# rlangefe/pygemma

Hardware: AMD Instinct MI355X
Metric: SNPs/sec (whole node) at n=10,000 c=5; K-eigendecomp wallclock (higher is better)
Workload: dtype i8x3->i32 MFMA (genotype codes exact, integer accumulation exact; U as 24-bit fixed point per eigenvector in three int8 planes) rotation + f64 Gram/sweeps (f32 rounding points of the reference)

## Files before the change

pygemma_amd/csrc/assoc.hip:

```cpp
#include "common.hpp"

#include <cmath>

namespace pg {

constexpr int NLAM = 11;
#ifndef PG_ASSOC_WPB
#define PG_ASSOC_WPB 2
#endif
constexpr int WPB = PG_ASSOC_WPB;
#define PG_MINV 1e-35f
#ifndef PG_FUSE_PQ_MAX
#define PG_FUSE_PQ_MAX 36
#endif
#ifndef PG_FUSE_PQR_MAX
#define PG_FUSE_PQR_MAX 28
#endif
#ifndef PG_PFD
#define PG_PFD 2
#endif
#ifndef PG_CHUNK_MIN_NP
#define PG_CHUNK_MIN_NP 80
#endif
#ifndef PG_SCAN_NV
#define PG_SCAN_NV 96
#endif
#ifndef PG_SWEEP_LDS_MIN_SLOTS
#define PG_SWEEP_LDS_MIN_SLOTS 3
#endif
#ifndef PG_PHENO_SPLIT_XE
#define PG_PHENO_SPLIT_XE 26
#endif
#ifndef PG_WAVES
#define PG_WAVES 2
#endif
#ifndef PG_ASSOC_FINAL_P
#define PG_ASSOC_FINAL_P 1
#endif
#ifndef PG_ASSOC_NEWTON_REUSE
#define PG_ASSOC_NEWTON_REUSE 1
#endif
#ifndef PG_REUSE_MAX_SLOTS
#define PG_REUSE_MAX_SLOTS 4
#endif

__host__ __device__ constexpr size_t assoc_sav_doubles(int sav_slots) { return sav_slots ? (size_t)2 * (2 * sav_slots + 1) * 64 : 0; }
__host__ __device__ constexpr size_t assoc_per_wave_bytes(int M, bool sweep_lds, int sav_slots, size_t evalout_bytes, int n_vals)
{
    return (((sweep_lds ? (size_t)3 * M * 8 : 0) + assoc_sav_doubles(sav_slots) * 8 + (size_t)NLAM * 2 * M * 8 + NLAM * evalout_bytes + 2 * NLAM * 4 +
             (size_t)n_vals * 4) + 15) & ~(size_t)15;
}

struct AssocParams {
    int n, npad, c, niter, nu, grid, rowf;
    long long p, ldx;
    const float *xr;
    const float *fixed;
    float *htab;
    double *fixg;
    double *t1tab;
    float *ldHtab;
    float lam11[NLAM];
    float logl_c;
    const int *leaf, *node, *level, *chunk;
    int n_leaf, n_level, n_chunk, n_vals;
    float *beta, *se, *tau, *lam;
    double *F;
    unsigned long long *stats;
    unsigned *trace;
    unsigned long long *passes;
    int lrt, nhalf;
    float ml_c;
    float *lalt, *lamalt;
    const double *xbuf;
    int xe, xcol;
};

struct EvalOut { float yPy, yPPy, yPPPy, trP, trPP, ld, Pxx_c, Pyx_c, sh, shh; };

__device__ __forceinline__ float hinv_f32(float lam, float d)
{
    const float x = __fadd_rn(__fmul_rn(lam, d), 1.0f);
    const float r0 = __builtin_amdgcn_rcpf(x);
    float r = __builtin_fmaf(__builtin_fmaf(-x, r0, 1.0f), r0, r0);
    if (__builtin_expect(!(x < 0x1p126f), 0)) r = __fdiv_rn(1.0f, x);
    return r;
}

__device__ __forceinline__ float np_logf(float x)
{
    const float p1 = 9.999999999999998702752e-01f, p2 = 2.112677543073053063722e+00f,
                p3 = 1.480000633576506585156e+00f, p4 = 3.808837741388407920751e-01f,
                p5 = 2.589979117907922693523e-02f;
    const float q1 = 2.612677543073109236779e+00f, q2 = 2.453006071784736363091e+00f,
                q3 = 9.864942958519418960339e-01f, q4 = 1.546476374983906719538e-01f,
                q5 = 5.875095403124574342950e-03f;
    if (__builtin_expect(!(x > 0.0f) || x == INFINITY, 0)) return (x != x) ? x : (x < 0.0f ? NAN : (x == 0.0f ? -INFINITY : x));
    unsigned u = __float_as_uint(x);
    int e = (int)((u >> 23) & 0xff) - 126;
    float m = __uint_as_float((u & 0x007fffffu) | 0x3f000000u);
    float ef = (float)e;
    if (m <= 0.70710678118f) { m = __fadd_rn(m, m); ef = __fsub_rn(ef, 1.0f); }
    float t = __fsub_rn(m, 1.0f);
    float den = fmaf(q5, t, q4);
    den = fmaf(den, t, q3); den = fmaf(den, t, q2); den = fmaf(den, t, q1); den = fmaf(den, t, 1.0f);
    float num = fmaf(p5, t, p4);
    num = fmaf(num, t, p3); num = fmaf(num, t, p2); num = fmaf(num, t, p1); num = fmaf(num, t, 0.0f);
    float poly = __fdiv_rn(num, den);
    return fmaf(ef, 0.693147180559945309417232121458176568f, poly);
}

__device__ __forceinline__ double bfly(double v)
{
#pragma unroll
// ... 136 lines not shown
        const bool b = (lane & s) != 0;
#pragma unroll
        for (int m = 0; m < NVP / (2 * s); m++) {
            const double keep = b ? v[2 * m + 1] : v[2 * m];
            const double send = b ? v[2 * m] : v[2 * m + 1];
            v[m] = keep + __shfl_xor(send, s, 64);
        }
    }
    double x = v[0];
#pragma unroll
    for (int s = NVP; s < 64; s <<= 1) x += __shfl_xor(x, s, 64);
    return x;
}

template <int C, int SL = 0>
__device__ __forceinline__ void scatter_entries(const double (&acc)[Shape<C>::NP], int lane, double (&out)[Shape<C>::SLOTS])
{
    constexpr int NV = Shape<C>::slot_nv(SL), NVP = next_pow2(NV);
    double t[NVP];
#pragma unroll
    for (int k = 0; k < NVP; k++) t[k] = (k < NV) ? acc[64 * SL + k] : 0.0;
    out[SL] = reduce_scatter<NVP>(t, lane);
    if constexpr (SL + 1 < Shape<C>::SLOTS) scatter_entries<C, SL + 1>(acc, lane, out);
}

template <int C> struct Own {
    int e[Shape<C>::SLOTS], r[Shape<C>::SLOTS], c[Shape<C>::SLOTS];
    bool valid[Shape<C>::SLOTS];
    __device__ __forceinline__ void init(int lane)
    {
#pragma unroll
        for (int sl = 0; sl < Shape<C>::SLOTS; sl++) {
            const int nv = Shape<C>::slot_nv(sl), k = lane % next_pow2(nv);
            valid[sl] = k < nv;
            e[sl] = valid[sl] ? 64 * sl + k : 0;
            int rr = 0;
            while ((rr + 1) * (rr + 2) / 2 <= e[sl]) rr++;
            r[sl] = rr; c[sl] = e[sl] - rr * (rr + 1) / 2;
        }
    }
};

template <int SLOTS>
__device__ __forceinline__ double gather(const double (&X)[SLOTS], int es)
{
    double v = __shfl(X[0], es & 63, 64);
#pragma unroll
    for (int sl = 1; sl < SLOTS; sl++) { const double w = __shfl(X[sl], es & 63, 64); v = ((es >> 6) == sl) ? w : v; }
    return v;
}

__device__ __forceinline__ void wave_lds_sync();

template <int C, int PW>
__device__ __forceinline__ void lane_sweeps(double (&P)[Shape<C>::SLOTS], double (&Q)[Shape<C>::SLOTS], double (&R)[Shape<C>::SLOTS],
                                            const Own<C> &own, double t1, double t2, int lane, EvalOut &o, double *piv)
{
    constexpr int M = Shape<C>::M, NP = Shape<C>::NP, SLOTS = Shape<C>::SLOTS;
    static_assert(PW == PW_P || PW == PW_PQ || PW == PW_PQR, "powers");
    constexpr bool DQ = (PW & 2) != 0, FULL = (PW & 4) != 0;
    constexpr bool VIA_LDS = Shape<C>::SWEEP_LDS;
    if (own.valid[0] && own.e[0] == 0) P[0] = dmaxf(P[0], PG_MINV);
    double trP = t1, trPP = t2, apiv = 1.0;
    for (int i = 1; i < M; i++) {
        const int q = i - 1, eqq = tri(q, q);
        double a, b = 0.0, e = 0.0;
        double ur[SLOTS], uc[SLOTS], vr[SLOTS], vc[SLOTS], wr[SLOTS], wc[SLOTS];
        bool act[SLOTS];
        if constexpr (VIA_LDS) {
#pragma unroll
            for (int sl = 0; sl < SLOTS; sl++)
                if (own.valid[sl] && own.c[sl] == q) {
                    piv[own.r[sl]] = P[sl];
                    if (DQ) piv[M + own.r[sl]] = Q[sl];
                    if (FULL) piv[2 * M + own.r[sl]] = R[sl];
                }
            wave_lds_sync();
            a = piv[q];
            if (DQ) b = piv[M + q];
            if (FULL) e = piv[2 * M + q];
#pragma unroll
            for (int sl = 0; sl < SLOTS; sl++) {
                act[sl] = own.valid[sl] && own.c[sl] >= i;
                const int rr = act[sl] ? own.r[sl] : q, cc = act[sl] ? own.c[sl] : q;
                ur[sl] = piv[rr]; uc[sl] = piv[cc];
                if (DQ) { vr[sl] = piv[M + rr]; vc[sl] = piv[M + cc]; }
                if (FULL) { wr[sl] = piv[2 * M + rr]; wc[sl] = piv[2 * M + cc]; }
            }
            wave_lds_sync();
        } else {
            a = gather<SLOTS>(P, eqq);
            if (DQ) b = gather<SLOTS>(Q, eqq);
            if (FULL) e = gather<SLOTS>(R, eqq);
#pragma unroll
            for (int sl = 0; sl < SLOTS; sl++) {
                act[sl] = own.valid[sl] && own.c[sl] >= i;
                const int er = act[sl] ? tri(own.r[sl], q) : 0, ec = act[sl] ? tri(own.c[sl], q) : 0;
                ur[sl] = gather<SLOTS>(P, er); uc[sl] = gather<SLOTS>(P, ec);
                if (DQ) { vr[sl] = gather<SLOTS>(Q, er); vc[sl] = gather<SLOTS>(Q, ec); }
                if (FULL) { wr[sl] = gather<SLOTS>(R, er); wc[sl] = gather<SLOTS>(R, ec); }
            }
        }
        if (lane == q) apiv = a;
        const double a2 = a * a, ia = -1.0 / a, ba2 = b / a2;
        if constexpr (FULL) {
            const double ba = b / a;
            trPP = (trPP + ba * ba) - 2 * (e / a);
            const double a3 = a2 * a, b2 = b * b;
            const double cR = (e / a2) - (b2 / a3);
#pragma unroll
            for (int sl = 0; sl < SLOTS; sl++)
                if (act[sl]) {
                    double s1 = fma(cR * uc[sl], ur[sl], R[sl]);
                    double s2 = fma(ia * uc[sl], wr[sl], 0.0); s2 = fma(ia * wc[sl], ur[sl], s2);
                    double s3 = fma(ia * vc[sl], vr[sl], 0.0);
                    double s4 = fma(ba2 * uc[sl], vr[sl], 0.0); s4 = fma(ba2 * vc[sl], ur[sl], s4);
                    double rn = ((s1 + s2) + s3) + s4;
                    if (own.r[sl] == i && own.c[sl] == i) rn = dmaxf(rn, PG_MINV);
                    R[sl] = rn;
                }
        }
        if constexpr (DQ) {
            trP = trP - b / a;
#pragma unroll
            for (int sl = 0; sl < SLOTS; sl++)
                if (act[sl]) {
                    double s1 = fma(ba2 * uc[sl], ur[sl], Q[sl]);
                    double s2 = fma(ia * uc[sl], vr[sl], 0.0); s2 = fma(ia * vc[sl], ur[sl], s2);
                    double qn = s1 + s2;
                    double pn = fma(ia * uc[sl], ur[sl], P[sl]);
                    if (own.r[sl] == i && own.c[sl] == i) { qn = dmaxf(qn, PG_MINV); pn = dmaxf(pn, PG_MINV); }
                    Q[sl] = qn; P[sl] = pn;
                }
        } else {
#pragma unroll
            for (int sl = 0; sl < SLOTS; sl++)
                if (act[sl]) {
                    double pn = fma(ia * uc[sl], ur[sl], P[sl]);
                    if (own.r[sl] == i && own.c[sl] == i) pn = dmaxf(pn, PG_MINV);
                    P[sl] = pn;
                }
        }
        if (i == M - 2) { o.Pxx_c = (float)gather<SLOTS>(P, tri(M - 2, M - 2)); o.Pyx_c = (float)gather<SLOTS>(P, tri(M - 1, M - 2)); }
    }
    const double lg = log(apiv);
    float ld = 0.0f;
    for (int q = 0; q < M - 1; q++) ld = (float)((double)ld + __shfl(lg, q, 64));
    o.yPy = (float)gather<SLOTS>(P, NP - 1);
    o.yPPy = DQ ? (float)gather<SLOTS>(Q, NP - 1) : 0.0f;
    o.yPPPy = FULL ? (float)gather<SLOTS>(R, NP - 1) : 0.0f;
    o.trP = DQ ? (float)trP : 0.0f;
    o.trPP = FULL ? (float)trPP : 0.0f;
    o.ld = ld;
    o.sh = (float)t1;
    o.shh = FULL ? (float)t2 : 0.0f;
}

template <int C> struct Elem {
    static constexpr int S4 = (C + 2 + 3) / 4;
    float4 row[S4];
    float x;
};
template <int C, bool HASX = true>
__device__ __forceinline__ void load_elem(const AssocParams &pr, const float *xrow, int i, Elem<C> &e)
{
    const float4 *src = reinterpret_cast<const float4 *>(pr.fixed + (size_t)i * pr.rowf);
#pragma unroll
    for (int k = 0; k < Elem<C>::S4; k++) e.row[k] = src[k];
    const int ic = min(i, pr.n - 1);
    e.x = HASX ? xrow[ic] : 0.0f;
}
constexpr int PFD = PG_PFD;
template <class E, int PF = PFD, class LoadF, class BodyF>
__device__ __forceinline__ void pipelined(int niter, LoadF &&ld, BodyF &&body)
{
    E buf[PF];
#pragma unroll
    for (int d = 0; d < PF; d++) ld(buf[d], d < niter ? d : niter - 1);
    for (int it = 0; it < niter; it += PF) {
#pragma unroll
        for (int d = 0; d < PF; d++) {
            if (it + d < niter) body(buf[d], it + d);
            const int nx = it + d + PF;
            ld(buf[d], nx < niter ? nx : niter - 1);
        }
    }
}
template <int C>
__device__ __forceinline__ void unpack_elem(const AssocParams &pr, const Elem<C> &e, int i, float &d, float (&col)[C + 2])
{
    float buf[4 * Elem<C>::S4];
#pragma unroll
    for (int k = 0; k < Elem<C>::S4; k++) {
        buf[4 * k] = e.row[k].x; buf[4 * k + 1] = e.row[k].y; buf[4 * k + 2] = e.row[k].z; buf[4 * k + 3] = e.row[k].w;
    }
    d = buf[0];
#pragma unroll
    for (int j = 0; j < C; j++) col[j] = buf[1 + j];
    col[C] = e.x;
    col[C + 1] = buf[C + 1];
// ... 113 lines not shown
        if constexpr (DR) slot_passes<C, 3, true, 0, EL>(pr, xrow, lam, lane, nullptr, R, t2);
    } else if constexpr (MASK == PW_PQR && Shape<C>::FUSE_PQR) {
        gram_pass<C, 7, true, EL>(pr, xrow, lam, lane, nullptr, P, Q, R, t1, t2);
    } else if constexpr (DP && DQ && Shape<C>::FUSE_PQ) {
        gram_pass<C, 3, true, EL>(pr, xrow, lam, lane, nullptr, P, Q, R, t1, t2);
        if constexpr (DR) gram_pass<C, 4, true, EL>(pr, xrow, lam, lane, nullptr, P, Q, R, t1, t2);
    } else {
        if constexpr (DP) gram_pass<C, 1, true, EL>(pr, xrow, lam, lane, nullptr, P, Q, R, t1, t2);
        if constexpr (DQ) gram_pass<C, 2, true, EL>(pr, xrow, lam, lane, nullptr, P, Q, R, t1, t2);
        if constexpr (DR) gram_pass<C, 4, true, EL>(pr, xrow, lam, lane, nullptr, P, Q, R, t1, t2);
    }
}

template <int C, int PW, class EL = WaldElem<C>>
__device__ __forceinline__ void eval_specific(const AssocParams &pr, typename EL::Row xrow, float lam, int lane, const Own<C> &own, EvalOut &o,
                                              double *piv)
{
    constexpr int SLOTS = Shape<C>::SLOTS;
    double P[SLOTS], Q[SLOTS], R[SLOTS], t1 = 0.0, t2 = 0.0;
#pragma unroll
    for (int sl = 0; sl < SLOTS; sl++) { Q[sl] = 0.0; R[sl] = 0.0; }
    gram_powers<C, PW, EL>(pr, xrow, lam, lane, P, Q, R, t1, t2);
    lane_sweeps<C, PW>(P, Q, R, own, t1, t2, lane, o, piv);
}

template <int C>
__global__ __launch_bounds__(64) void setup_tabs_kernel(AssocParams pr)
{
    constexpr int NP = Shape<C>::NP, SLOTS = Shape<C>::SLOTS;
    extern __shared__ float smem_f[];
    const int t = blockIdx.x, lane = threadIdx.x;
    const float lam = pr.lam11[t];
    Own<C> own;
    own.init(lane);
    double P[SLOTS], Q[SLOTS], R[SLOTS], t1 = 0.0, t2 = 0.0;
    if constexpr (Shape<C>::CHUNKED) {
        double tq = 0.0;
        slot_passes<C, 1, false>(pr, nullptr, lam, lane, pr.htab + (size_t)t * pr.npad, P, t1);
        slot_passes<C, 2, false>(pr, nullptr, lam, lane, nullptr, Q, tq);
    } else if constexpr (Shape<C>::FUSE_PQ) {
        gram_pass<C, 3, false>(pr, nullptr, lam, lane, pr.htab + (size_t)t * pr.npad, P, Q, R, t1, t2);
    } else {
        gram_pass<C, 1, false>(pr, nullptr, lam, lane, pr.htab + (size_t)t * pr.npad, P, Q, R, t1, t2);
        gram_pass<C, 2, false>(pr, nullptr, lam, lane, nullptr, P, Q, R, t1, t2);
    }
#pragma unroll
    for (int sl = 0; sl < SLOTS; sl++)
        if (own.valid[sl]) {
            pr.fixg[((size_t)t * 2 + 0) * NP + own.e[sl]] = P[sl];
            pr.fixg[((size_t)t * 2 + 1) * NP + own.e[sl]] = Q[sl];
        }
    float ldH = device_logdet_H(pr, lam, lane, smem_f);
    if (lane == 0) { pr.t1tab[t] = t1; pr.ldHtab[t] = ldH; }
}

template <int C, int GG>
__device__ __forceinline__ void scan_accumulate(const AssocParams &pr, const float *xrow, int t0, int lane, double *xent)
{
    constexpr int M = Shape<C>::M, NV = GG * 2 * M;
    constexpr int NV0 = NV < 64 ? NV : 64, NV1 = NV > 64 ? NV - 64 : 0;
    constexpr int NVP0 = next_pow2(NV0), NVP1 = next_pow2(NV1 > 0 ? NV1 : 1);
    static_assert(NV <= 128, "scan group too large");
    double acc[NV0 == 64 ? 64 + NVP1 : NVP0];
#pragma unroll
    for (int k = 0; k < (NV0 == 64 ? 64 + NVP1 : NVP0); k++) acc[k] = 0.0;
    struct SE { Elem<C> e; float h[GG]; };
    pipelined<SE>(pr.niter, [&](SE &q, int it) {
        const int i = it * 64 + lane;
        load_elem<C>(pr, xrow, i, q.e);
#pragma unroll
        for (int g = 0; g < GG; g++) q.h[g] = pr.htab[(size_t)(t0 + g) * pr.npad + i];
    }, [&](const SE &q, int it) {
        const int i = it * 64 + lane;
        float d, colf[M];
        unpack_elem<C>(pr, q.e, i, d, colf);
        const double xd = (double)colf[C];
        double z[M];
#pragma unroll
        for (int k = 0; k <= C; k++) z[k] = xd * (double)colf[k];
        z[C + 1] = (double)colf[C + 1] * xd;
#pragma unroll
        for (int g = 0; g < GG; g++) {
            const double hd = (double)q.h[g];
            const double h2 = hd * hd;
#pragma unroll
            for (int k = 0; k <= C + 1; k++) {
                acc[g * 2 * M + k] = fma(hd, z[k], acc[g * 2 * M + k]);
                acc[g * 2 * M + M + k] = fma(h2, z[k], acc[g * 2 * M + M + k]);
            }
        }
    });
    {
        double t[NVP0];
#pragma unroll
        for (int k = 0; k < NVP0; k++) t[k] = acc[k];
        const double tot = reduce_scatter<NVP0>(t, lane);
        const int idx = lane % NVP0;
        if (idx < NV0 && lane < NVP0) xent[t0 * 2 * M + idx] = tot;
    }
    if constexpr (NV1 > 0) {
        double t[NVP1];
#pragma unroll
        for (int k = 0; k < NVP1; k++) t[k] = acc[64 + k];
        const double tot = reduce_scatter<NVP1>(t, lane);
        const int idx = lane % NVP1;
        if (idx < NV1 && lane < NVP1) xent[t0 * 2 * M + 64 + idx] = tot;
// ... 120 lines not shown
        if (fabs(fblk) < fabs(fcur)) {
            xpre = xcur; xcur = xblk; xblk = xpre;
            fpre = fcur; fcur = fblk; fblk = fpre;
        }
        delta = (xtol + rtol * fabs(xcur)) / 2;
        sbis = (xblk - xcur) / 2;
        if (fcur == 0 || fabs(sbis) < delta) return xcur;
        if (fabs(spre) > delta && fabs(fcur) < fabs(fpre)) {
            if (xpre == xblk) {
                stry = -fcur * (xcur - xpre) / (fcur - fpre);
            } else {
                dpre = (fpre - fcur) / (xpre - xcur);
                dblk = (fblk - fcur) / (xblk - xcur);
                stry = -fcur * (fblk * dblk - fpre * dpre) / (dblk * dpre * (fblk - fpre));
            }
            double lim = 3 * fabs(sbis) - delta;
            double mn = fabs(spre) < lim ? fabs(spre) : lim;
            if (2 * fabs(stry) < mn) { spre = scur; scur = stry; }
            else { spre = sbis; scur = sbis; }
        } else { spre = sbis; scur = sbis; }
        xpre = xcur; fpre = fcur;
        if (fabs(scur) > delta) xcur += scur;
        else xcur += (sbis > 0 ? delta : -delta);
        fcur = f(xcur);
    }
    return xcur;
}

template <class Eval>
__device__ __forceinline__ float newton_dev(const AssocParams &pr, float lroot, float l0, float l1, Eval &&eval)
{
    int iteration = 0;
    for (;;) {
        EvalOut e;
        eval(lroot, e);
        const float d1 = d1_f(pr, lroot, e.yPy, e.yPPy, e.trP);
        const float d2 = d2_f(pr, lroot, e.yPy, e.yPPy, e.yPPPy, e.trP, e.trPP);
        const float ratio = __fdiv_rn(d1, d2);
        const bool any_nan = (ratio != ratio) || (d1 != d1) || (d2 != d2);
        const float sr = (float)((ratio > 0) - (ratio < 0)), s1 = (float)((d1 > 0) - (d1 < 0)), s2 = (float)((d2 > 0) - (d2 < 0));
        if (!any_nan && sr * s1 * s2 <= 0.0f) break;
        const float lnew = __fsub_rn(lroot, ratio);
        const float r_eps = (float)(fabs((double)__fsub_rn(lnew, lroot)) / fabs((double)lroot));
        if (lnew < l0) break;
        if (lnew > l1) break;
        if (isnan(lnew) || isinf(lnew)) break;
        lroot = lnew;
        if ((double)r_eps < 1e-5 || iteration > 100) break;
        iteration++;
    }
    return lroot;
}

template <int C, bool LRT, bool PHENO = false>
__global__ __launch_bounds__(64 * WPB, PG_WAVES) void assoc_kernel(AssocParams pr)
{
    constexpr int M = Shape<C>::M, NP = Shape<C>::NP, SLOTS = Shape<C>::SLOTS;
    extern __shared__ unsigned char smem[];
    const int wave = threadIdx.x >> 6, lane = threadIdx.x & 63;
    static_assert(!(PHENO && LRT), "the multi-phenotype search has no LRT");
    const long long g = (long long)blockIdx.x * WPB + wave;
    if (g >= pr.p) return;
    constexpr size_t piv_bytes = Shape<C>::SWEEP_LDS ? (size_t)3 * M * 8 : 0;
    constexpr bool REUSE = Shape<C>::NEWTON_REUSE;
    unsigned char *base = smem + (size_t)wave * assoc_per_wave_bytes(M, Shape<C>::SWEEP_LDS, Shape<C>::SAV_SLOTS, sizeof(EvalOut), pr.n_vals);
    double *piv = reinterpret_cast<double *>(base);
    base += piv_bytes;
    double *sav = reinterpret_cast<double *>(base) + lane;
    base += assoc_sav_doubles(Shape<C>::SAV_SLOTS) * 8;
    double *xent = reinterpret_cast<double *>(base);
    EvalOut *evs = reinterpret_cast<EvalOut *>(base + (size_t)NLAM * 2 * M * 8);
    float *d1s = reinterpret_cast<float *>(evs + NLAM);
    float *lls = d1s + NLAM;
    float *vals = lls + NLAM;
    const float *xrow = pr.xr + (size_t)g * pr.ldx;

    Own<C> own;
    own.init(lane);
    if constexpr (PHENO) {
        const double *src = pr.xbuf + (size_t)g * NLAM * 2 * pr.xe;
        for (int j = lane; j < NLAM * 2 * M; j += 64) {
            const int tp = j / M, k = j - tp * M;
            xent[j] = src[(size_t)tp * pr.xe + (k <= C ? k : pr.xcol)];
        }
    } else {
        scan_all<C, 0>(pr, xrow, lane, xent);
    }
    wave_lds_sync();
    for (int t = 0; t < NLAM; t++) {
        double P[SLOTS], Q[SLOTS], R[SLOTS];
        const double *fp = pr.fixg + ((size_t)t * 2 + 0) * NP, *fq = pr.fixg + ((size_t)t * 2 + 1) * NP;
        const double *xe = xent + t * 2 * M;
#pragma unroll
        for (int sl = 0; sl < SLOTS; sl++) {
            const int r = own.r[sl], c = own.c[sl];
            const bool isx = (r == C) || (r == C + 1 && c == C);
            const int k = (r == C) ? c : C + 1;
            P[sl] = isx ? xe[k] : fp[own.e[sl]];
            Q[sl] = isx ? xe[M + k] : fq[own.e[sl]];
            R[sl] = 0.0;
        }
        EvalOut e;
        lane_sweeps<C, PW_PQ>(P, Q, R, own, pr.t1tab[t], 0.0, lane, e, piv);
        if (lane == 0) {
            evs[t] = e;
            d1s[t] = d1_f(pr, pr.lam11[t], e.yPy, e.yPPy, e.trP);
            lls[t] = logl_f(pr, e.yPy, pr.ldHtab[t], e.ld);
        }
    }
    wave_lds_sync();
    float best_l = lls[0], best_lambda;
    EvalOut best_e;
    if (best_l < lls[NLAM - 1]) { best_l = lls[NLAM - 1]; best_lambda = pr.lam11[NLAM - 1]; best_e = evs[NLAM - 1]; }
    else { best_lambda = pr.lam11[0]; best_e = evs[0]; }
    unsigned n_fast = 0, n_full = 0, n_ponly = 0, n_reuse = 0;
    constexpr int PW_FINAL = PG_ASSOC_FINAL_P ? PW_P : PW_PQ;
    if (pr.grid) {
        for (int t = 0; t < NLAM - 1; t++)
            if (lls[t] > best_l) { best_l = lls[t]; best_lambda = pr.lam11[t]; best_e = evs[t]; }
    } else {
        for (int k = 0; k < NLAM - 1; k++) {
            const float f0 = d1s[k], f1 = d1s[k + 1];
            if (__builtin_signbit(f0) == __builtin_signbit(f1)) continue;
            const float l0 = pr.lam11[k], l1 = pr.lam11[k + 1];
            float sav_lam0 = NAN, sav_lam1 = NAN;
            unsigned sav_next = 0;
            double root = brentq_dev(
                [&](double x) -> double {
                    EvalOut e;
                    const float lf = (float)x;
                    if constexpr (REUSE) {
                        double P[SLOTS], Q[SLOTS], R[SLOTS], t1 = 0.0, t2 = 0.0;
#pragma unroll
                        for (int sl = 0; sl < SLOTS; sl++) R[sl] = 0.0;
                        gram_powers<C, PW_PQ>(pr, xrow, lf, lane, P, Q, R, t1, t2);
                        double *sv = sav + sav_next * Shape<C>::SAV_STRIDE;
#pragma unroll
                        for (int sl = 0; sl < SLOTS; sl++) { sv[64 * sl] = P[sl]; sv[64 * (SLOTS + sl)] = Q[sl]; }
                        sv[64 * 2 * SLOTS] = t1;
                        if (sav_next) sav_lam1 = lf; else sav_lam0 = lf;
                        sav_next ^= 1u;
                        lane_sweeps<C, PW_PQ>(P, Q, R, own, t1, t2, lane, e, piv);
                    } else {
                        eval_specific<C, PW_PQ>(pr, xrow, lf, lane, own, e, piv);
                    }
                    n_fast++;
                    return (double)d1_f(pr, lf, e.yPy, e.yPPy, e.trP);
                },
                (double)l0, (double)l1, (double)f0, (double)f1);
            bool first = true;
            const float lroot = newton_dev(pr, (float)root, l0, l1, [&](float lf, EvalOut &e) {
                if constexpr (REUSE) {
                    const unsigned lb = __float_as_uint(lf);
                    const int hit = !(first && lf == lf) ? -1 : (lb == __float_as_uint(sav_lam0)) ? 0 : (lb == __float_as_uint(sav_lam1)) ? 1 : -1;
                    first = false;
                    double P[SLOTS], Q[SLOTS], R[SLOTS], t1 = 0.0, t2 = 0.0;
                    if (hit >= 0) {
                        const double *sv = sav + hit * Shape<C>::SAV_STRIDE;
#pragma unroll
                        for (int sl = 0; sl < SLOTS; sl++) { P[sl] = sv[64 * sl]; Q[sl] = sv[64 * (SLOTS + sl)]; }
                        t1 = sv[64 * 2 * SLOTS];
                        gram_powers<C, PW_R>(pr, xrow, lf, lane, P, Q, R, t1, t2);
// ... 28 lines not shown
            if (f0 != f0 || f1 != f1) continue;
            const float s0 = (float)((f0 > 0) - (f0 < 0)), s1 = (float)((f1 > 0) - (f1 < 0));
            if (!(s0 * s1 < 0.0f)) continue;
            double p0 = brentq_dev(
                [&](double x) -> double {
                    EvalOut e;
                    const float lf = (float)x;
                    eval_specific<C, PW_PQ>(pr, xrow, lf, lane, own, e, piv);
                    n_fast++;
                    return (double)ml_d1_f(pr, lf, e.yPy, e.yPPy, e.sh);
                },
                (double)pr.lam11[k], (double)pr.lam11[k + 1], (double)f0, (double)f1, 5000);
            double pn = p0;
            for (int itr = 0; itr < 10; itr++) {
                EvalOut e;
                const float lf = (float)p0;
                eval_specific<C, PW_PQR>(pr, xrow, lf, lane, own, e, piv);
                n_full++;
                const float fval = ml_d1_f(pr, lf, e.yPy, e.yPPy, e.sh);
                if (fval == 0.0f) { pn = p0; break; }
                const float fder = ml_d2_f(pr, lf, e.yPy, e.yPPy, e.yPPPy, e.sh, e.shh);
                if (fder == 0.0f) { pn = p0; break; }
                pn = p0 - (double)__fdiv_rn(fval, fder);
                if (fabs(pn - p0) <= 1.48e-8 + 1e-5 * fabs(p0)) break;
                p0 = pn;
            }
            if (ml_l == ml_l) {
                EvalOut e;
                const float lf = (float)pn;
                eval_specific<C, PW_FINAL>(pr, xrow, lf, lane, own, e, piv);
                n_fast++;
                if (PW_FINAL == PW_P) n_ponly++;
                const float l = ml_logl_f(pr, e.yPy, device_logdet_H(pr, lf, lane, vals));
                if (l != l || l > ml_l) { ml_l = l; ml_lam = lf; }
            }
        }
        if (lane == 0) { pr.lalt[g] = ml_l; pr.lamalt[g] = ml_lam; }
    }
    if (lane == 0) {
        const float b = __fdiv_rn(best_e.Pyx_c, best_e.Pxx_c);
        const float pxx = (PG_MINV > best_e.Pxx_c) ? PG_MINV : best_e.Pxx_c;
        const float sb = (float)(__dsqrt_rn((double)best_e.yPy) / ((double)sqrtf(pxx) * __dsqrt_rn((double)(pr.nu))));
        const float ta = __fdiv_rn((float)pr.nu, best_e.yPy);
        const double t = (double)__fdiv_rn(b, sb);
        pr.beta[g] = b; pr.se[g] = sb; pr.tau[g] = ta; pr.lam[g] = best_lambda; pr.F[g] = t * t;
        if (pr.stats) { atomicAdd(&pr.stats[0], (unsigned long long)n_fast); atomicAdd(&pr.stats[1], (unsigned long long)n_full); }
        if (pr.trace) pr.trace[g] = n_fast | (n_full << 16);
        if (pr.passes) {
            const unsigned long long np = (unsigned long long)(n_fast + n_full - n_reuse);
            atomicAdd(&pr.passes[0], np); atomicAdd(&pr.passes[1], np - n_ponly);
            atomicAdd(&pr.passes[2], (unsigned long long)n_full); atomicAdd(&pr.passes[3], (unsigned long long)n_reuse);
        }
    }
}

#if defined(PG_ASSOC_PART) && (PG_ASSOC_PART == 6 || PG_ASSOC_PART == 7)
struct GxeRows { const float *x, *xe; };
template <int CS> struct GxeVals {
    static constexpr int S4 = (CS + 2 + 3) / 4;
    float4 row[S4];
    float x, xe;
};
template <int C> struct GxeElem {
    static constexpr int CS = C - 1;
    using E = GxeVals<CS>;
    using Row = GxeRows;
    template <bool HASX>
    static __device__ __forceinline__ void load(const AssocParams &pr, Row r, int i, E &e)
    {
        const float4 *src = reinterpret_cast<const float4 *>(pr.fixed + (size_t)i * pr.rowf);
#pragma unroll
        for (int k = 0; k < E::S4; k++) e.row[k] = src[k];
        const int ic = min(i, pr.n - 1);
        e.x = r.x[ic];
        e.xe = r.xe[ic];
    }
    static __device__ __forceinline__ void unpack(const AssocParams &pr, const E &e, int i, float &d, float (&col)[C + 2])
    {
        float buf[4 * E::S4];
#pragma unroll
        for (int k = 0; k < E::S4; k++) {
            buf[4 * k] = e.row[k].x; buf[4 * k + 1] = e.row[k].y; buf[4 * k + 2] = e.row[k].z; buf[4 * k + 3] = e.row[k].w;
        }
        d = buf[0];
#pragma unroll
        for (int j = 0; j < CS; j++) col[j] = buf[1 + j];
        col[CS] = e.x;
        col[CS + 1] = e.xe;
        col[CS + 2] = buf[CS + 1];
    }
};
template <int CS> struct GxeShape {
    static constexpr int C = CS + 1, NE = 2 * CS + 5;
    static constexpr int PWS = NE > PG_PHENO_SPLIT_XE ? 1 : 2;
    static constexpr int G0 = (Shape<C>::SCAN_NV - NE) / (PWS * NE), G = G0 < 1 ? 1 : (G0 > NLAM ? NLAM : G0);
};
__host__ __device__ constexpr size_t gxe_per_wave_bytes(int M, bool sweep_lds, int NE, size_t evalout_bytes, int n_vals)
{
    return (((sweep_lds ? (size_t)3 * M * 8 : 0) + (size_t)NLAM * 2 * NE * 8 + NLAM * evalout_bytes + 2 * NLAM * 4 + (size_t)n_vals * 4) + 15) & ~(size_t)15;
}

template <int CS, int GG, int PWS, int PW0>
__device__ __forceinline__ void gxe_scan_accumulate(const AssocParams &pr, GxeRows xr, int t0, int lane, double *out)
{
    using EL = GxeElem<CS + 1>;
    constexpr int M = CS + 3, NE = GxeShape<CS>::NE, NV = GG * PWS * NE;
// ... 594 lines not shown
    fdist_sf_kernel<<<(unsigned)((count + 255) / 256), 256, 0, ctx->stream>>>(count, F, dfd, pval);
    PG_HIP(hipGetLastError());
    return PG_OK;
}

extern "C" int pg_transpose_dev(pg_ctx *ctx, int64_t n, int64_t p, const float *X, int64_t ldX, float *Xr, int64_t ldx)
{
    PG_REQUIRE(ctx && X && Xr && n > 0 && p > 0 && ldx >= n && ldX >= p, "pg_transpose_dev: bad arguments");
    PG_HIP(hipSetDevice(ctx->device));
    dim3 grid((unsigned)((p + 31) / 32), (unsigned)((ldx + 31) / 32));
    transpose_kernel<<<grid, 256, 0, ctx->stream>>>(n, p, X, ldX, Xr, ldx);
    PG_HIP(hipGetLastError());
    return PG_OK;
}

static void fill_params(pg_ctx *ctx, int64_t n, int c, int grid, AssocParams &pr)
{
    pr.n = (int)n; pr.npad = (int)((n + 63) / 64 * 64); pr.c = c; pr.niter = pr.npad / 64;
    pr.nu = (int)(n - c - 1); pr.grid = grid ? 1 : 0; pr.rowf = ((c + 2 + 3) / 4) * 4;
    for (int k = -5; k <= 5; k++) pr.lam11[k + 5] = (float)pow(10.0, (double)(float)k);
    {
        const int ctot = c + 1;
        float r = (float)((0.5 * (double)(n - ctot)) * std::log(0.5 * (double)(n - ctot) / M_PI));
        r = (float)((double)r - (0.5 * (double)(n - ctot)));
        pr.logl_c = r;
    }
    pr.nhalf = (int)(n / 2);
    {
        float r = (float)((double)(n / 2) * std::log((double)n / (2.0 * M_PI)));
        pr.ml_c = r - (float)(n / 2);
    }
    pr.leaf = ctx->plan.d_leaf; pr.node = ctx->plan.d_node; pr.level = ctx->plan.d_level; pr.chunk = ctx->plan.d_chunk;
    pr.n_leaf = ctx->plan.n_leaf; pr.n_level = ctx->plan.n_level; pr.n_chunk = ctx->plan.n_chunk;
    pr.n_vals = ctx->plan.n_leaf + ctx->plan.n_node;
}

static int assoc_run(pg_ctx *ctx, int64_t n, int c, int64_t p, const float *d, const float *Wr, int64_t ldw, const float *yr,
                     const float *Xr, int64_t ldx, int grid, float *beta, float *se, float *tau, float *lambda, double *F,
                     unsigned long long *stats_dev, bool lrt, float *lalt, float *lamalt)
{
    PG_HIP(hipSetDevice(ctx->device));
    int rc = build_npsum_plan(ctx, n);
    if (rc) return rc;

    AssocParams pr{};
    fill_params(ctx, n, c, grid, pr);
    pr.p = p; pr.ldx = ldx; pr.xr = Xr;
    const int M = c + 2, NP = M * (M + 1) / 2;
    rc = ensure(ctx, &ctx->fixed, &ctx->fixed_bytes, (size_t)pr.npad * pr.rowf * 4);
    if (rc) return rc;
    const size_t off_fixg = ((size_t)NLAM * pr.npad * 4 + 255) & ~(size_t)255;
    const size_t off_t1 = off_fixg + (size_t)NLAM * 2 * NP * 8;
    const size_t off_ldh = off_t1 + NLAM * 8;
    rc = ensure(ctx, &ctx->tabs, &ctx->tabs_bytes, off_ldh + NLAM * 4 + 256);
    if (rc) return rc;
    if (!ctx->stats) PG_HIP(hipMalloc(&ctx->stats, 16));
    pr.fixed = (const float *)ctx->fixed;
    pr.htab = (float *)ctx->tabs;
    pr.fixg = (double *)((char *)ctx->tabs + off_fixg);
    pr.t1tab = (double *)((char *)ctx->tabs + off_t1);
    pr.ldHtab = (float *)((char *)ctx->tabs + off_ldh);
    pr.lrt = lrt ? 1 : 0;
    pr.lalt = lalt; pr.lamalt = lamalt;
    pr.beta = beta; pr.se = se; pr.tau = tau; pr.lam = lambda; pr.F = F;
    pr.stats = stats_dev;
    pr.trace = lrt ? nullptr : ctx->eval_trace;
    pr.passes = lrt ? nullptr : ctx->pass_stats;

    build_fixed_kernel<<<(pr.npad + 255) / 256, 256, 0, ctx->stream>>>(pr.n, pr.npad, c, (int)ldw, pr.rowf, d, Wr, yr, (float *)ctx->fixed);
    PG_HIP(hipGetLastError());
    return launch_assoc_any(ctx, pr);
}

extern "C" int pg_assoc_dev(pg_ctx *ctx, int64_t n, int c, int64_t p, const float *d, const float *Wr, const float *yr,
                            const float *Xr, int64_t ldx, int grid, float *beta, float *se, float *tau, float *lambda,
                            double *F, double *pval, unsigned long long *stats_dev)
{
    PG_REQUIRE(ctx && d && Wr && yr && Xr && beta && se && tau && lambda && F, "pg_assoc_dev: NULL argument");
    PG_REQUIRE(n >= 2 && n < (1LL << 30) && p >= 0 && ldx >= n, "pg_assoc_dev: bad shape n=%lld p=%lld ldx=%lld", (long long)n, (long long)p, (long long)ldx);
    if (c < 1 || c > PG_MAX_COVARIATES) {
        set_error("pg_assoc_dev: c=%d covariates not supported by this build (1..%d)", c, PG_MAX_COVARIATES);
        return PG_ENOTSUP;
    }
    PG_REQUIRE(n - c - 1 > 0, "pg_assoc_dev: n - c - 1 must be positive");
    if (p == 0) return PG_OK;
    int rc = assoc_run(ctx, n, c, p, d, Wr, c, yr, Xr, ldx, grid, beta, se, tau, lambda, F, stats_dev, false, nullptr, nullptr);
    if (rc) return rc;
    if (pval) return pg_fdist_sf_dev(ctx, p, F, (double)(n - c - 1), pval);
    return PG_OK;
}

extern "C" int pg_assoc_warm(pg_ctx *ctx, int64_t n, int c)
{
    PG_REQUIRE(ctx && n >= 2 && n < (1LL << 30), "pg_assoc_warm: bad arguments");
    if (c < 1 || c > PG_MAX_COVARIATES) {
        set_error("pg_assoc_warm: c=%d covariates not supported by this build (1..%d)", c, PG_MAX_COVARIATES);
        return PG_ENOTSUP;
    }
    PG_HIP(hipSetDevice(ctx->device));
    int rc = build_npsum_plan(ctx, n);
    if (rc) return rc;
    const int npad = (int)((n + 63) / 64 * 64), rowf = ((c + 2 + 3) / 4) * 4, M = c + 2, NP = M * (M + 1) / 2;
    rc = ensure(ctx, &ctx->fixed, &ctx->fixed_bytes, (size_t)npad * rowf * 4);
    if (rc) return rc;
    const size_t off_fixg = ((size_t)NLAM * npad * 4 + 255) & ~(size_t)255;
    rc = ensure(ctx, &ctx->tabs, &ctx->tabs_bytes, off_fixg + (size_t)NLAM * 2 * NP * 8 + NLAM * 8 + NLAM * 4 + 256);
    if (rc) return rc;
    if (!ctx->stats) PG_HIP(hipMalloc(&ctx->stats, 16));
    return PG_OK;
}

extern "C" int pg_assoc_set_eval_trace(pg_ctx *ctx, unsigned *trace_dev)
{
    PG_REQUIRE(ctx, "pg_assoc_set_eval_trace: NULL ctx");
    ctx->eval_trace = trace_dev;
    return PG_OK;
}

extern "C" int pg_assoc_set_pass_stats(pg_ctx *ctx, unsigned long long *dev4)
{
    PG_REQUIRE(ctx, "pg_assoc_set_pass_stats: NULL ctx");
    ctx->pass_stats = dev4;
    return PG_OK;
}

struct PhenoLayout {
    int npad, rowf, NP, tpad_max;
    long long ptile;
    size_t off_htab, off_fixg, off_t1, off_ldh, off_xbuf, bytes;
};
static PhenoLayout pheno_layout(int64_t n, int c, int t, int64_t p)
{
    PhenoLayout L{};
    auto up = [](size_t v) { return (v + 255) & ~(size_t)255; };
    L.npad = (int)((n + 63) / 64 * 64); L.rowf = ((c + 2 + 3) / 4) * 4; L.NP = (c + 2) * (c + 3) / 2;
    const int tc = t < PHENO_CHUNK ? t : PHENO_CHUNK;
    L.tpad_max = 1;
    while (L.tpad_max < tc) L.tpad_max <<= 1;
    const size_t per_snp = (size_t)NLAM * 2 * (c + 1 + L.tpad_max) * 8;
    const long long cap = (long long)((256u << 20) / per_snp);
    L.ptile = p < cap ? p : (cap < 1024 ? 1024 : cap);
    if (L.ptile > p) L.ptile = p;
    L.off_htab = up((size_t)PHENO_CHUNK * L.npad * L.rowf * 4);
    L.off_fixg = L.off_htab + up((size_t)NLAM * L.npad * 4);
    L.off_t1 = L.off_fixg + up((size_t)PHENO_CHUNK * NLAM * 2 * L.NP * 8);
    L.off_ldh = L.off_t1 + up(NLAM * 8);
    L.off_xbuf = L.off_ldh + up(NLAM * 4);
    L.bytes = L.off_xbuf + up((size_t)L.ptile * per_snp);
    return L;
}

extern "C" int pg_assoc_pheno_dev(pg_ctx *ctx, int64_t n, int c, int64_t p, int t, const float *d, const float *Wr,
                                  const float *Yr, int64_t ldy, const float *Xr, int64_t ldx, int grid,
                                  float *beta, float *se, float *tau, float *lambda, double *F, double *pval,
                                  unsigned long long *stats_dev)
{
    PG_REQUIRE(ctx && d && Wr && Yr && Xr && beta && se && tau && lambda && F, "pg_assoc_pheno_dev: NULL argument");
    PG_REQUIRE(n >= 2 && n < (1LL << 30) && p >= 0 && ldx >= n, "pg_assoc_pheno_dev: bad shape n=%lld p=%lld ldx=%lld",
               (long long)n, (long long)p, (long long)ldx);
    if (c < 1 || c > PG_MAX_COVARIATES) {
        set_error("pg_assoc_pheno_dev: c=%d covariates not supported by this build (1..%d)", c, PG_MAX_COVARIATES);
        return PG_ENOTSUP;
    }
    PG_REQUIRE(n - c - 1 > 0, "pg_assoc_pheno_dev: n - c - 1 must be positive");
    PG_REQUIRE(t >= 1 && ldy >= n, "pg_assoc_pheno_dev: bad phenotypes t=%d ldy=%lld (n=%lld)", t, (long long)ldy, (long long)n);
    if (p == 0) return PG_OK;
    PG_HIP(hipSetDevice(ctx->device));
    int rc = build_npsum_plan(ctx, n);
    if (rc) return rc;
    const PhenoLayout L = pheno_layout(n, c, t, p);
    rc = ensure(ctx, &ctx->pheno, &ctx->pheno_bytes, L.bytes);
    if (rc) return rc;
    char *base = (char *)ctx->pheno;
    float *fixed = (float *)base;
    double *fixg = (double *)(base + L.off_fixg), *xbuf = (double *)(base + L.off_xbuf);

    AssocParams pr{};
// ... 273 lines not shown
```

Baseline: 1.892 million.

## Hoist SNP-independent sweep pivots into per-lambda decade table for assoc grid

Precomputes, once per lambda in the fixed-table kernel, the covariate-only pivot coefficients and P/Q columns of the sweep into a device table. Each SNP's 11-lambda grid evaluation then updates only a one-column vector per lambda using packed lanes (several lambdas per wave), skipping the full triangular sweep. This cuts per-SNP double-precision shuffle and FMA work in the grid phase. It adds a global table read per lambda, changes the rounding order slightly, and adds optional timing-stamp instrumentation behind a macro.

Result: faster. 1.945 million, median of 6 (+2.8%).

```diff
diff --git a/pygemma_amd/csrc/assoc.hip b/pygemma_amd/csrc/assoc.hip
--- a/pygemma_amd/csrc/assoc.hip
+++ b/pygemma_amd/csrc/assoc.hip
@@ -43,6 +43,11 @@
 #ifndef PG_REUSE_MAX_SLOTS
 #define PG_REUSE_MAX_SLOTS 4
 #endif
+#ifndef PG_ASSOC_DECADE_HOIST
+#define PG_ASSOC_DECADE_HOIST 1
+#endif
+
+__host__ __device__ constexpr size_t assoc_dtab_doubles(int c) { return (size_t)c * (c + 2) * 4 + 8; }
 
 __host__ __device__ constexpr size_t assoc_sav_doubles(int sav_slots) { return sav_slots ? (size_t)2 * (2 * sav_slots + 1) * 64 : 0; }
 __host__ __device__ constexpr size_t assoc_per_wave_bytes(int M, bool sweep_lds, int sav_slots, size_t evalout_bytes, int n_vals)
@@ -60,6 +65,7 @@
     double *fixg;
     double *t1tab;
     float *ldHtab;
+    double *dtab;
     float lam11[NLAM];
     float logl_c;
     const int *leaf, *node, *level, *chunk;
@@ -302,17 +308,18 @@
 
 __device__ __forceinline__ void wave_lds_sync();
 
-template <int C, int PW>
+template <int C, int PW, bool REC = false>
 __device__ __forceinline__ void lane_sweeps(double (&P)[Shape<C>::SLOTS], double (&Q)[Shape<C>::SLOTS], double (&R)[Shape<C>::SLOTS],
-                                            const Own<C> &own, double t1, double t2, int lane, EvalOut &o, double *piv)
+                                            const Own<C> &own, double t1, double t2, int lane, EvalOut &o, double *piv, double *rec = nullptr)
 {
     constexpr int M = Shape<C>::M, NP = Shape<C>::NP, SLOTS = Shape<C>::SLOTS;
     static_assert(PW == PW_P || PW == PW_PQ || PW == PW_PQR, "powers");
+    static_assert(!REC || PW == PW_PQ, "the decade table holds P and Q");
     constexpr bool DQ = (PW & 2) != 0, FULL = (PW & 4) != 0;
     constexpr bool VIA_LDS = Shape<C>::SWEEP_LDS;
     if (own.valid[0] && own.e[0] == 0) P[0] = dmaxf(P[0], PG_MINV);
     double trP = t1, trPP = t2, apiv = 1.0;
-    for (int i = 1; i < M; i++) {
+    for (int i = 1; i < (REC ? M - 1 : M); i++) {
         const int q = i - 1, eqq = tri(q, q);
         double a, b = 0.0, e = 0.0;
         double ur[SLOTS], uc[SLOTS], vr[SLOTS], vc[SLOTS], wr[SLOTS], wc[SLOTS];
@@ -353,6 +360,14 @@
         }
         if (lane == q) apiv = a;
         const double a2 = a * a, ia = -1.0 / a, ba2 = b / a2;
+        if constexpr (REC) {
+            double *rq = rec + (size_t)q * M * 4;
+            if (lane < M) { rq[4 * lane] = ia; rq[4 * lane + 1] = ba2; }
+            if (lane <= q) { rq[4 * lane + 2] = 0.0; rq[4 * lane + 3] = 0.0; }
+#pragma unroll
+            for (int sl = 0; sl < SLOTS; sl++)
+                if (own.valid[sl] && own.c[sl] == q && own.r[sl] > q) { rq[4 * own.r[sl] + 2] = P[sl]; rq[4 * own.r[sl] + 3] = Q[sl]; }
+        }
         if constexpr (FULL) {
             const double ba = b / a;
             trPP = (trPP + ba * ba) - 2 * (e / a);
@@ -395,7 +410,13 @@
     }
     const double lg = log(apiv);
     float ld = 0.0f;
-    for (int q = 0; q < M - 1; q++) ld = (float)((double)ld + __shfl(lg, q, 64));
+    for (int q = 0; q < (REC ? M - 2 : M - 1); q++) ld = (float)((double)ld + __shfl(lg, q, 64));
+    if constexpr (REC) {
+        const double pyy = gather<SLOTS>(P, NP - 1), qyy = gather<SLOTS>(Q, NP - 1);
+        double *tail = rec + (size_t)C * M * 4;
+        if (lane == 0) { tail[0] = trP; tail[1] = (double)ld; tail[2] = pyy; tail[3] = qyy; }
+        return;
+    }
     o.yPy = (float)gather<SLOTS>(P, NP - 1);
     o.yPPy = DQ ? (float)gather<SLOTS>(Q, NP - 1) : 0.0f;
     o.yPPPy = FULL ? (float)gather<SLOTS>(R, NP - 1) : 0.0f;
@@ -615,6 +636,16 @@
         }
     float ldH = device_logdet_H(pr, lam, lane, smem_f);
     if (lane == 0) { pr.t1tab[t] = t1; pr.ldHtab[t] = ldH; }
+    if constexpr (PG_ASSOC_DECADE_HOIST && C >= 1) {
+        __shared__ double piv_s[Shape<C>::SWEEP_LDS ? 3 * Shape<C>::M : 1];
+        if (pr.dtab) {
+            double *rec = pr.dtab + (size_t)t * assoc_dtab_doubles(C);
+            EvalOut e;
+            lane_sweeps<C, PW_PQ, true>(P, Q, R, own, t1, 0.0, lane, e, piv_s, rec);
+            double *tail = rec + (size_t)C * Shape<C>::M * 4;
+            if (lane == 0) { tail[4] = t1; tail[5] = (double)ldH; tail[6] = (double)lam; tail[7] = 0.0; }
+        }
+    }
 }
 
 template <int C, int GG>
@@ -841,6 +872,68 @@
     return lroot;
 }
 
+#if defined(PG_ASSOC_STAMPS) && !defined(PG_ASSOC_PART)
+__device__ long long g_assoc_stamps[1024 * 4];
+#define ASSOC_STAMP(slot)                                                                                       \
+    do {                                                                                                        \
+        const long long sq_ = pr.p >= 1024 ? pr.p / 1024 : 1, sr_ = g / sq_;                                    \
+        if (lane == 0 && sr_ < 1024 && g == sr_ * sq_)                                                          \
+            g_assoc_stamps[sr_ * 4 + slot] = (long long)__builtin_amdgcn_s_memtime();                           \
+    } while (0)
+#else
+#define ASSOC_STAMP(slot) do { } while (0)
+#endif
+
+template <int C>
+__device__ __forceinline__ void decade_lanes(const AssocParams &pr, const double *xent, int lane, EvalOut *evs, float *d1s, float *lls)
+{
+    constexpr int M = Shape<C>::M, G = 64 / M;
+    static_assert(C >= 1 && G >= 2, "decade_lanes: one covariate step at least, two lambdas per round at least");
+    const int tl = lane / M, k = lane - tl * M;
+    for (int t0 = 0; t0 < NLAM; t0 += G) {
+        const bool on = tl < G && t0 + tl < NLAM;
+        const int g = on ? tl : 0, t = t0 + g, base = g * M;
+        const double2 *tab = reinterpret_cast<const double2 *>(pr.dtab + (size_t)t * assoc_dtab_doubles(C));
+        double P = xent[t * 2 * M + k], Q = xent[t * 2 * M + M + k];
+#pragma unroll
+        for (int q = 0; q < C; q++) {
+            const double2 s = tab[(q * M + k) * 2], w = tab[(q * M + k) * 2 + 1];
+            const double ia = s.x, ba2 = s.y;
+            const double xp = __shfl(P, base + q, 64), xq = __shfl(Q, base + q, 64);
+            const double ur = (k == C + 1) ? w.x : xp, uc = (k < C) ? w.x : xp;
+            const double vr = (k == C + 1) ? w.y : xq, vc = (k < C) ? w.y : xq;
+            double s1 = fma(ba2 * uc, ur, Q);
+            double s2 = fma(ia * uc, vr, 0.0); s2 = fma(ia * vc, ur, s2);
+            double qn = s1 + s2;
+            double pn = fma(ia * uc, ur, P);
+            if (q == C - 1 && k == C) { qn = dmaxf(qn, PG_MINV); pn = dmaxf(pn, PG_MINV); }
+            if (k > q) { Q = qn; P = pn; }
+        }
+        const double a = __shfl(P, base + C, 64), b = __shfl(Q, base + C, 64);
+        const double u = __shfl(P, base + C + 1, 64), v = __shfl(Q, base + C + 1, 64);
+        const double2 z0 = tab[C * M * 2], z1 = tab[C * M * 2 + 1], z2 = tab[C * M * 2 + 2], z3 = tab[C * M * 2 + 3];
+        const double t1 = z2.x;
+        const float ldH = (float)z2.y, lam = (float)z3.x;
+        EvalOut e;
+        e.Pxx_c = (float)a; e.Pyx_c = (float)u;
+        const double a2 = a * a, ia = -1.0 / a, ba2 = b / a2;
+        const double trP = z0.x - b / a;
+        double s1 = fma(ba2 * u, u, z1.y);
+        double s2 = fma(ia * u, v, 0.0); s2 = fma(ia * v, u, s2);
+        const double qn = dmaxf(s1 + s2, PG_MINV);
+        const double pn = dmaxf(fma(ia * u, u, z1.x), PG_MINV);
+        e.yPy = (float)pn; e.yPPy = (float)qn; e.yPPPy = 0.0f;
+        e.trP = (float)trP; e.trPP = 0.0f;
+        e.ld = (float)((double)(float)z0.y + log(a));
+        e.sh = (float)t1; e.shh = 0.0f;
+        if (on && k == 0) {
+            evs[t] = e;
+            d1s[t] = d1_f(pr, lam, e.yPy, e.yPPy, e.trP);
+            lls[t] = logl_f(pr, e.yPy, ldH, e.ld);
+        }
+    }
+}
+
 template <int C, bool LRT, bool PHENO = false>
 __global__ __launch_bounds__(64 * WPB, PG_WAVES) void assoc_kernel(AssocParams pr)
 {
@@ -850,6 +943,7 @@
     static_assert(!(PHENO && LRT), "the multi-phenotype search has no LRT");
     const long long g = (long long)blockIdx.x * WPB + wave;
     if (g >= pr.p) return;
+    ASSOC_STAMP(0);
     constexpr size_t piv_bytes = Shape<C>::SWEEP_LDS ? (size_t)3 * M * 8 : 0;
     constexpr bool REUSE = Shape<C>::NEWTON_REUSE;
     unsigned char *base = smem + (size_t)wave * assoc_per_wave_bytes(M, Shape<C>::SWEEP_LDS, Shape<C>::SAV_SLOTS, sizeof(EvalOut), pr.n_vals);
@@ -876,7 +970,10 @@
         scan_all<C, 0>(pr, xrow, lane, xent);
     }
     wave_lds_sync();
-    for (int t = 0; t < NLAM; t++) {
+    ASSOC_STAMP(1);
+    constexpr bool HOIST = PG_ASSOC_DECADE_HOIST && !PHENO && C >= 1 && 64 / M >= 2;
+    if constexpr (HOIST) decade_lanes<C>(pr, xent, lane, evs, d1s, lls);
+    else for (int t = 0; t < NLAM; t++) {
         double P[SLOTS], Q[SLOTS], R[SLOTS];
         const double *fp = pr.fixg + ((size_t)t * 2 + 0) * NP, *fq = pr.fixg + ((size_t)t * 2 + 1) * NP;
         const double *xe = xent + t * 2 * M;
@@ -897,6 +994,7 @@
             lls[t] = logl_f(pr, e.yPy, pr.ldHtab[t], e.ld);
         }
     }
+    ASSOC_STAMP(2);
     wave_lds_sync();
     float best_l = lls[0], best_lambda;
     EvalOut best_e;
@@ -1031,6 +1129,7 @@
             atomicAdd(&pr.passes[2], (unsigned long long)n_full); atomicAdd(&pr.passes[3], (unsigned long long)n_reuse);
         }
     }
+    ASSOC_STAMP(3);
 }
 
 #if defined(PG_ASSOC_PART) && (PG_ASSOC_PART == 6 || PG_ASSOC_PART == 7)
@@ -1731,7 +1830,8 @@
     const size_t off_fixg = ((size_t)NLAM * pr.npad * 4 + 255) & ~(size_t)255;
     const size_t off_t1 = off_fixg + (size_t)NLAM * 2 * NP * 8;
     const size_t off_ldh = off_t1 + NLAM * 8;
-    rc = ensure(ctx, &ctx->tabs, &ctx->tabs_bytes, off_ldh + NLAM * 4 + 256);
+    const size_t off_dtab = (off_ldh + NLAM * 4 + 255) & ~(size_t)255;
+    rc = ensure(ctx, &ctx->tabs, &ctx->tabs_bytes, off_dtab + NLAM * assoc_dtab_doubles(c) * 8 + 256);
     if (rc) return rc;
     if (!ctx->stats) PG_HIP(hipMalloc(&ctx->stats, 16));
     pr.fixed = (const float *)ctx->fixed;
@@ -1739,6 +1839,7 @@
     pr.fixg = (double *)((char *)ctx->tabs + off_fixg);
     pr.t1tab = (double *)((char *)ctx->tabs + off_t1);
     pr.ldHtab = (float *)((char *)ctx->tabs + off_ldh);
+    pr.dtab = (double *)((char *)ctx->tabs + off_dtab);
     pr.lrt = lrt ? 1 : 0;
     pr.lalt = lalt; pr.lamalt = lamalt;
     pr.beta = beta; pr.se = se; pr.tau = tau; pr.lam = lambda; pr.F = F;
@@ -1783,7 +1884,8 @@
     rc = ensure(ctx, &ctx->fixed, &ctx->fixed_bytes, (size_t)npad * rowf * 4);
     if (rc) return rc;
     const size_t off_fixg = ((size_t)NLAM * npad * 4 + 255) & ~(size_t)255;
-    rc = ensure(ctx, &ctx->tabs, &ctx->tabs_bytes, off_fixg + (size_t)NLAM * 2 * NP * 8 + NLAM * 8 + NLAM * 4 + 256);
+    rc = ensure(ctx, &ctx->tabs, &ctx->tabs_bytes,
+                ((off_fixg + (size_t)NLAM * 2 * NP * 8 + NLAM * 8 + NLAM * 4 + 255) & ~(size_t)255) + NLAM * assoc_dtab_doubles(c) * 8 + 256);
     if (rc) return rc;
     if (!ctx->stats) PG_HIP(hipMalloc(&ctx->stats, 16));
     return PG_OK;
@@ -1802,6 +1904,13 @@
     ctx->pass_stats = dev4;
     return PG_OK;
 }
+
+#ifdef PG_ASSOC_STAMPS
+extern "C" int pgx_assoc_stamps(long long *out4096)
+{
+    return hipMemcpyFromSymbol(out4096, HIP_SYMBOL(pg::g_assoc_stamps), sizeof(long long) * 4096) == hipSuccess ? 0 : -1;
+}
+#endif
 
 struct PhenoLayout {
     int npad, rowf, NP, tpad_max;
```
